# RajaeeKh/TriNerfLet

Measured on AMD Instinct MI355X. Metric: train rays/sec (whole node), higher is better.
Workload: dtype f16; 1 GPU; base: 3x32ch x 2048^2 planes, bior6.8 scale 32, hidden 64, 60000 rays/step/GPU, solid-sphere occupancy r=0.8 (re-imposed after each refresh), fp16 planes + fp16 MFMA MLP, fp32 masters, Adam+L1; GT colours = an analytic function of the ray direction (synthetic.target_colors), not a second seeded field's render; sample_budget_M=4769546, parallelism=ray-dp1

## Files before the change

include/trinerflet_hip.h:

```cpp
#ifndef TRINERFLET_HIP_H
#define TRINERFLET_HIP_H

#include <stdint.h>

#ifdef __cplusplus
extern "C" {
#endif

#define TNL_API __attribute__((visibility("default")))

TNL_API int tnl_abi_version(void);


TNL_API int tnl_near_far_from_aabb(const float *rays_o, const float *rays_d, const float *aabb,
                                   uint32_t N, float min_near, float *nears, float *fars,
                                   void *stream);

TNL_API int tnl_sph_from_ray(const float *rays_o, const float *rays_d, float radius, uint32_t N,
                             float *coords, void *stream);

TNL_API int tnl_morton3D(const int32_t *coords, uint32_t N, int32_t *indices, void *stream);

TNL_API int tnl_morton3D_invert(const int32_t *indices, uint32_t N, int32_t *coords, void *stream);

TNL_API int tnl_packbits(const float *grid, uint32_t N, float density_thresh, uint8_t *bitfield,
                         void *stream);
TNL_API int tnl_packbits_dev(const float *grid, uint32_t N, float density_thresh, const float *mean_density_dev,
                             uint8_t *bitfield, void *stream);

TNL_API int tnl_occupancy_bounds(const uint8_t *bitfield, uint32_t bytes_per_cascade, uint32_t cascades,
                                 int32_t *bounds, void *stream);
TNL_API int tnl_occupancy_row_extents(const uint8_t *bitfield, uint32_t bytes_per_cascade, uint32_t cascades, uint32_t H,
                                      float bound, uint32_t R, int32_t *ext, void *stream);

TNL_API int tnl_occupied_box(const uint8_t *bitfield, uint32_t bytes_per_cascade, uint32_t cascades, uint32_t H,
                             float bound, int32_t *bounds_scratch, float *box, void *stream);
TNL_API int tnl_clip_fars(const float *rays_o, const float *rays_d, const float *fars, const float *box, uint32_t N,
                          float *fars_out, void *stream);

TNL_API uint32_t tnl_march_rays_train_workspace(uint32_t N);
TNL_API uint32_t tnl_march_rays_train_workspace_rec(uint32_t N, uint32_t max_steps);

TNL_API int tnl_march_rays_train(const float *rays_o, const float *rays_d, const uint8_t *grid,
                                 float bound, float dt_gamma, uint32_t max_steps, uint32_t N,
                                 uint32_t C, uint32_t H, uint32_t M, const float *nears,
                                 const float *fars, float *xyzs, float *dirs, float *deltas,
                                 int32_t *rays, int32_t *counter, const float *noises,
                                 int32_t *workspace, uint32_t workspace_words, void *stream);
TNL_API int tnl_march_rays_train_binned(const float *rays_o, const float *rays_d, const uint8_t *grid,
                                 float bound, float dt_gamma, uint32_t max_steps, uint32_t N,
                                 uint32_t C, uint32_t H, uint32_t M, const float *nears,
                                 const float *fars, float *xyzs, float *dirs, float *deltas,
                                 int32_t *rays, int32_t *counter, const float *noises,
                                 int32_t *workspace, uint32_t workspace_words, uint32_t R, void *sort_workspace, void *stream);

TNL_API int tnl_march_count_form(int form);

TNL_API int tnl_march_emit_cap(int blocks);
TNL_API int tnl_plane_grad_fill_cap(int blocks);

TNL_API int tnl_composite_rays_train_forward(const float *sigmas, const float *rgbs,
                                             const float *deltas, const int32_t *rays, uint32_t M,
                                             uint32_t N, float T_thresh, float *weights_sum,
                                             float *depth, float *image, void *stream);

TNL_API int tnl_composite_rays_train_backward(const float *grad_weights_sum, const float *grad_image,
                                              const float *sigmas, const float *rgbs,
                                              const float *deltas, const int32_t *rays,
                                              const float *weights_sum, const float *image,
                                              uint32_t M, uint32_t N, float T_thresh,
                                              float *grad_sigmas, float *grad_rgbs, void *stream);

TNL_API int tnl_march_rays(uint32_t n_alive, uint32_t n_step, const int32_t *rays_alive,
                           const float *rays_t, const float *rays_o, const float *rays_d,
                           float bound, float dt_gamma, uint32_t max_steps, uint32_t C, uint32_t H,
                           const uint8_t *grid, const float *nears, const float *fars, float *xyzs,
                           float *dirs, float *deltas, const float *noises, void *stream);

TNL_API int tnl_composite_rays(uint32_t n_alive, uint32_t n_step, float T_thresh,
                               int32_t *rays_alive, float *rays_t, const float *sigmas,
                               const float *rgbs, const float *deltas, float *weights_sum,
                               float *depth, float *image, void *stream);

TNL_API int tnl_compact_rays(const int32_t *rays_alive, uint32_t n_alive, int32_t *rays_alive_out,
                             int32_t *n_out, int32_t *workspace, void *stream);

TNL_API int tnl_sh_encode_forward(const float *inputs, float *outputs, uint32_t B, uint32_t D,
                                  uint32_t C, float *dy_dx, void *stream);
TNL_API int tnl_sh_encode_backward(const float *grad, const float *inputs, uint32_t B, uint32_t D,
                                   uint32_t C, const float *dy_dx, float *grad_inputs, void *stream);


TNL_API int tnl_idwt_level_forward(const float *x, const float *yh, uint32_t S, uint32_t n,
                                   int wave, float *out, void *stream);

TNL_API int tnl_idwt_level_forward_half(const float *x, const float *yh, uint32_t S, uint32_t n,
                                        int wave, void *out_half, void *stream);

TNL_API int tnl_idwt_level_backward(const float *dout, uint32_t S, uint32_t n, int wave, float *dx,
                                    float *dyh, void *stream);

TNL_API int tnl_idwt_level_backward_adam(const float *dout, uint32_t S, uint32_t n, int wave, float *dx,
                                         float *p, float *m, float *v, float *ll_p, float *ll_m,
                                         float *ll_v, float step_size, float bias2_sqrt, float beta1,
                                         float beta2, float eps, float inv_scale,
                                         const float *inv_scale_dev, float l1_coef,
                                         const float *found_inf, float *abs_sum, void *stream);

TNL_API int tnl_planes_to_texel_major(const float *planes_cm, uint32_t C, uint32_t R, int half_out,
                                      void *planes_tm, void *stream);
TNL_API int tnl_planes_to_texel_major_win(const float *planes_cm, uint32_t C, uint32_t R, int half_out,
                                          void *planes_tm, const int32_t *roi, void *stream);
TNL_API int tnl_planes_half_to_texel_major(const void *planes_cm_half, uint32_t C, uint32_t R,
                                           void *planes_tm_half, void *stream);
TNL_API int tnl_planes_to_channel_major(const float *grad_tm, uint32_t C, uint32_t R, float *grad_cm,
                                        void *stream);

TNL_API int tnl_triplane_sample_forward(const void *planes_tm, int half_in, const float *xyz,
                                        float bound, uint32_t N, uint32_t C, uint32_t R, float *feats,
                                        void *stream);
TNL_API int tnl_triplane_sample_backward(const float *grad_feats, const float *xyz, float bound,
                                         uint32_t N, uint32_t C, uint32_t R, float *grad_tm,
                                         void *stream);

TNL_API int tnl_grid_sample_tm_forward(const void *planes_tm, int half_in, const float *grid, uint32_t N, uint32_t C,
                                       uint32_t CG, uint32_t R, float *feats, void *stream);
TNL_API int tnl_grid_sample_tm_backward(const void *planes_tm, int half_in, const float *grid,
                                        const float *grad_feats, uint32_t N, uint32_t C, uint32_t CG, uint32_t R,
                                        float *grad_tm, float *grad_grid, void *stream);

TNL_API uint32_t tnl_field_packed_bytes(uint32_t C, uint32_t Hd, uint32_t Hc);
TNL_API int tnl_field_pack(const float *W0, const float *W1, const float *W2, const float *W3,
                           const float *W4, uint32_t C, uint32_t Hd, uint32_t Hc, void *packed,
                           void *stream);
TNL_API uint64_t tnl_field_feats_save_bytes(uint32_t M, uint32_t C, uint32_t Hd);
TNL_API int tnl_field_forward(const void *planes_tm, int half_in, const float *xyz, const float *dirs,
                              float bound, uint32_t M, uint32_t C, uint32_t R, uint32_t Hd,
                              uint32_t Hc, const void *packed, float *sigma, float *rgb,
                              void *feats_save, const int32_t *m_actual, void *stream);
TNL_API uint64_t tnl_field_backward_workspace(uint32_t M, uint32_t C, uint32_t Hd, uint32_t Hc);
TNL_API int tnl_field_backward(const float *grad_sigma, const float *grad_rgb, const float *sigma,
                               const float *rgb, const void *feats_save, const float *xyz,
                               const float *dirs, float bound, uint32_t M, uint32_t C, uint32_t R,
                               uint32_t Hd, uint32_t Hc, const void *packed, float *grad_tm,
                               float *gradW, void *workspace, const int32_t *m_actual, void *dfeat_half,
                               void *stream);

TNL_API uint64_t tnl_plane_grad_binned_workspace(uint32_t M, uint32_t R);
TNL_API int tnl_plane_grad_binned(const void *dfeat_half, const float *xyz, float bound, uint32_t M,
                                  const int32_t *m_actual, uint32_t C, uint32_t R, float grad_scale,
                                  float *grad_out, int channel_major, int32_t *nonfinite_flag,
                                  void *workspace, void *stream);

TNL_API int tnl_plane_grad_sort_layout(uint32_t M, uint32_t R, int64_t *out);
TNL_API int tnl_plane_grad_sort(const float *xyz, float bound, uint32_t M, const int32_t *m_actual, uint32_t R,
                                void *workspace, void *stream);
TNL_API int tnl_plane_grad_sort_counted(const float *xyz, float bound, uint32_t M, const int32_t *m_actual,
                                        uint32_t R, void *workspace, void *stream);
TNL_API int tnl_plane_grad_reduce(const void *dfeat_half, const float *xyz, float bound, uint32_t M, uint32_t C,
                                  uint32_t R,
                                  float grad_scale, float *grad_out, int channel_major, int32_t *nonfinite_flag,
                                  const int32_t *roi, const void *workspace, void *stream);

TNL_API int tnl_idwt_level_forward_half_roi(const float *x, const float *yh, uint32_t S, uint32_t n, int wave,
                                            void *out_half, const int32_t *roi, void *stream);
TNL_API int tnl_planes_half_to_texel_major_roi(const void *planes_roi_half, uint32_t C, uint32_t R,
                                               void *planes_tm_half, const int32_t *roi, void *stream);
TNL_API int tnl_plane_grad_binned_roi(const void *dfeat_half, const float *xyz, float bound, uint32_t M,
                                      const int32_t *m_actual, uint32_t C, uint32_t R, float grad_scale,
                                      float *grad_out, int channel_major, int32_t *nonfinite_flag,
                                      const int32_t *roi, void *workspace, void *stream);
TNL_API int tnl_idwt_level_backward_roi(const float *dout_roi, uint32_t S, uint32_t n, int wave, float *dx,
                                        float *dyh, const int32_t *roi, void *stream);

TNL_API int tnl_adam_l1_step(float *p, float *grad, float *m, float *v, uint64_t n, float step_size,
                             float bias2_sqrt, float beta1, float beta2, float eps, float inv_scale,
                             const float *inv_scale_dev, float l1_coef, const float *found_inf,
                             float *abs_sum, int zero_grad, void *stream);
TNL_API int tnl_adam_l1_step_dev(float *p, float *grad, float *m, float *v, uint64_t n, float lr,
                                 const float *opt_step_dev, float beta1, float beta2, float eps, float inv_scale,
                                 const float *inv_scale_dev, float l1_coef, const float *found_inf,
// ... 122 lines not shown
```

trinerflet_amd/build.py:

```python
import glob
import os
import subprocess
import sys
from concurrent.futures import ThreadPoolExecutor

HERE = os.path.dirname(os.path.abspath(__file__))
CSRC = os.path.join(HERE, "csrc")
OBJ = os.path.join(HERE, "csrc", "_obj")
LIB = os.path.join(HERE, "libtrinerflet_hip.so")
HIPCC = os.environ.get("HIPCC", "/opt/rocm/bin/hipcc")
ARCH = "gfx950"
COMMON = ["--offload-arch=" + ARCH, "-O3", "-fPIC", "-std=c++17", "-fvisibility=hidden",
          "-Wall", "-Wno-unused-function", "-I", os.path.join(HERE, "..", "include")]
COMMON += os.environ.get("TNL_HIPCC_FLAGS", "").split()
MFMA_VGPR = ["-mllvm", "-amdgpu-mfma-vgpr-form=1"]
NO_SLP = ["-fno-slp-vectorize"]
PER_FILE = {"raymarch.hip": ["-ffp-contract=off"], "rays.hip": ["-ffp-contract=off"],
            "field_bwd.hip": MFMA_VGPR,
            "field_bwd_rows.hip": MFMA_VGPR + ["-mllvm", "-amdgpu-sched-strategy=max-ilp"], "field.hip": MFMA_VGPR, "scatter.hip": MFMA_VGPR,
            "render.hip": MFMA_VGPR + NO_SLP, "field_h128.hip": MFMA_VGPR + NO_SLP + ["-mllvm", "-amdgpu-sched-strategy=max-ilp"]}
for _spec in filter(None, os.environ.get("TNL_HIPCC_FILE_FLAGS", "").split(";")):
    _name, _flags = _spec.split(":", 1)
    PER_FILE[_name.strip()] = PER_FILE.get(_name.strip(), []) + _flags.split()
INCLUDES = {"field_h128.hip": ["field.hip"]}


def _newer(src, dst, extra=()):
    if not os.path.exists(dst):
        return True
    t = os.path.getmtime(dst)
    return any(os.path.getmtime(p) > t for p in (src, *extra))


def build(verbose=False, force=False):
    os.makedirs(OBJ, exist_ok=True)
    headers = glob.glob(os.path.join(CSRC, "*.h")) + glob.glob(os.path.join(HERE, "..", "include", "*.h"))
    srcs = sorted(glob.glob(os.path.join(CSRC, "*.hip")))
    jobs = []
    objs = []
    for s in srcs:
        o = os.path.join(OBJ, os.path.basename(s)[:-4] + ".o")
        objs.append(o)
        if force or _newer(s, o, headers + [os.path.join(CSRC, d) for d in INCLUDES.get(os.path.basename(s), [])]):
            jobs.append([HIPCC, *COMMON, *PER_FILE.get(os.path.basename(s), []), "-c", s, "-o", o])

    def run(cmd):
        if verbose:
            print(" ".join(cmd), flush=True)
        r = subprocess.run(cmd, capture_output=True, text=True)
        if r.returncode != 0:
            raise RuntimeError("hipcc failed:\n" + " ".join(cmd) + "\n" + r.stdout + r.stderr)
        if verbose and r.stderr.strip():
            print(r.stderr)

    with ThreadPoolExecutor(max_workers=4) as ex:
        list(ex.map(run, jobs))
    if jobs or not os.path.exists(LIB):
        run([HIPCC, "--offload-arch=" + ARCH, "-shared", "-fPIC", "-o", LIB, *objs])
    return LIB


if __name__ == "__main__":
    print(build(verbose=True, force="--force" in sys.argv))
```

trinerflet_amd/nerf/renderer.py:

```python
import math

import numpy as np
import torch
import torch.nn as nn

from .. import _lib as L
from .. import raymarching


def sample_pdf(bins, weights, n_samples, det=False):
    pdf = weights + 1e-5
    pdf = pdf / pdf.sum(-1, keepdim=True)
    cdf = torch.cat([torch.zeros_like(pdf[..., :1]), torch.cumsum(pdf, -1)], -1)
    if det:
        u = torch.linspace(0.5 / n_samples, 1.0 - 0.5 / n_samples, steps=n_samples, device=weights.device)
        u = u.expand(*cdf.shape[:-1], n_samples)
    else:
        u = torch.rand(*cdf.shape[:-1], n_samples, device=weights.device)
    u = u.contiguous()
    hi = torch.searchsorted(cdf, u, right=True)
    lo = (hi - 1).clamp(min=0)
    hi = hi.clamp(max=cdf.shape[-1] - 1)
    c_lo, c_hi = torch.gather(cdf, -1, lo), torch.gather(cdf, -1, hi)
    b_lo, b_hi = torch.gather(bins, -1, lo), torch.gather(bins, -1, hi)
    span = c_hi - c_lo
    span = torch.where(span < 1e-5, torch.ones_like(span), span)
    return b_lo + (u - c_lo) / span * (b_hi - b_lo)


class NeRFRenderer(nn.Module):
    def __init__(self, bound=1, cuda_ray=False, density_scale=1, min_near=0.2, density_thresh=0.01, bg_radius=-1,
                 **kwargs):
        super().__init__()
        self.bound = bound
        self.cascade = 1 + math.ceil(math.log2(bound))
        self.grid_size = 128
        self.density_scale = density_scale
        self.min_near = min_near
        self.density_thresh = density_thresh
        self.bg_radius = bg_radius
        self._march_count = None
        self._march_window = None
        self.use_occupancy_window = True
        self._occ_window_key = None
        self._occ_window = None
        aabb_train = torch.FloatTensor([-bound, -bound, -bound, bound, bound, bound])
        self.register_buffer('aabb_train', aabb_train)
        self.register_buffer('aabb_infer', aabb_train.clone())
        self.cuda_ray = cuda_ray
        if cuda_ray:
            self.register_buffer('density_grid', torch.zeros([self.cascade, self.grid_size ** 3]))
            self.register_buffer('density_bitfield',
                                 torch.zeros(self.cascade * self.grid_size ** 3 // 8, dtype=torch.uint8))
            self.mean_density = 0
            self.iter_density = 0
            self.register_buffer('step_counter', torch.zeros(16, 2, dtype=torch.int32))
            self.mean_count = 0
            self.local_step = 0
        self._morton_xyz = None

    def forward(self, x, d):
        raise NotImplementedError()

    def density(self, x):
        raise NotImplementedError()

    def color(self, x, d, mask=None, **kwargs):
        raise NotImplementedError()

    def reset_extra_state(self):
        if not self.cuda_ray:
            return
        self.density_grid.zero_()
        self.mean_density = 0
        self.iter_density = 0
        self.step_counter.zero_()
        self.mean_count = 0
        self.local_step = 0

    def run(self, rays_o, rays_d, num_steps=128, upsample_steps=128, bg_color=None, perturb=False, **kwargs):
        prefix = rays_o.shape[:-1]
        rays_o = rays_o.contiguous().view(-1, 3)
        rays_d = rays_d.contiguous().view(-1, 3)
        N, device = rays_o.shape[0], rays_o.device
        aabb = self.aabb_train if self.training else self.aabb_infer
        nears, fars = raymarching.near_far_from_aabb(rays_o, rays_d, aabb, self.min_near)
        nears, fars = nears.unsqueeze(-1), fars.unsqueeze(-1)
        z_vals = torch.linspace(0.0, 1.0, num_steps, device=device).unsqueeze(0).expand(N, num_steps)
        z_vals = nears + (fars - nears) * z_vals
        sample_dist = (fars - nears) / num_steps
        if perturb:
            z_vals = z_vals + (torch.rand(z_vals.shape, device=device) - 0.5) * sample_dist
        xyzs = rays_o.unsqueeze(-2) + rays_d.unsqueeze(-2) * z_vals.unsqueeze(-1)
        xyzs = torch.min(torch.max(xyzs, aabb[:3]), aabb[3:])
        dens = self.density(xyzs.reshape(-1, 3))
        sigma = dens['sigma'].view(N, num_steps)
        geo = dens['geo_feat'].view(N, num_steps, -1)
        if upsample_steps > 0:
            with torch.no_grad():
                d0 = z_vals[..., 1:] - z_vals[..., :-1]
                d0 = torch.cat([d0, sample_dist * torch.ones_like(d0[..., :1])], dim=-1)
                a0 = 1 - torch.exp(-d0 * self.density_scale * sigma)
                w0 = a0 * torch.cumprod(torch.cat([torch.ones_like(a0[..., :1]), 1 - a0 + 1e-15], dim=-1), dim=-1)[..., :-1]
                z_mid = z_vals[..., :-1] + 0.5 * d0[..., :-1]
                new_z = sample_pdf(z_mid, w0[:, 1:-1], upsample_steps, det=not self.training).detach()
                new_xyzs = rays_o.unsqueeze(-2) + rays_d.unsqueeze(-2) * new_z.unsqueeze(-1)
                new_xyzs = torch.min(torch.max(new_xyzs, aabb[:3]), aabb[3:])
            new_dens = self.density(new_xyzs.reshape(-1, 3))
            z_vals, order = torch.sort(torch.cat([z_vals, new_z], dim=1), dim=1)
            xyzs = torch.gather(torch.cat([xyzs, new_xyzs], dim=1), 1, order.unsqueeze(-1).expand(-1, -1, 3))
            sigma = torch.gather(torch.cat([sigma, new_dens['sigma'].view(N, upsample_steps)], dim=1), 1, order)
            geo = torch.cat([geo, new_dens['geo_feat'].view(N, upsample_steps, -1)], dim=1)
            geo = torch.gather(geo, 1, order.unsqueeze(-1).expand(-1, -1, geo.shape[-1]))
        deltas = z_vals[..., 1:] - z_vals[..., :-1]
        deltas = torch.cat([deltas, sample_dist * torch.ones_like(deltas[..., :1])], dim=-1)
        alphas = 1 - torch.exp(-deltas * self.density_scale * sigma)
        alphas_shifted = torch.cat([torch.ones_like(alphas[..., :1]), 1 - alphas + 1e-15], dim=-1)
        weights = alphas * torch.cumprod(alphas_shifted, dim=-1)[..., :-1]
        dirs = rays_d.view(-1, 1, 3).expand_as(xyzs)
        mask = weights > 1e-4
        rgbs = self.color(xyzs.reshape(-1, 3), dirs.reshape(-1, 3), mask=mask.reshape(-1),
                          geo_feat=geo.reshape(-1, geo.shape[-1]))
        rgbs = rgbs.view(N, -1, 3)
        weights_sum = weights.sum(dim=-1)
        ori_z_vals = ((z_vals - nears) / (fars - nears)).clamp(0, 1)
        depth = torch.sum(weights * ori_z_vals, dim=-1)
        image = torch.sum(weights.unsqueeze(-1) * rgbs, dim=-2)
        if bg_color is None:
            bg_color = 1
        image = image + (1 - weights_sum).unsqueeze(-1) * bg_color
        return {'depth': depth.view(*prefix), 'image': image.view(*prefix, 3), 'weights_sum': weights_sum}

    def run_cuda(self, rays_o, rays_d, dt_gamma=0, bg_color=None, perturb=False, force_all_rays=False,
                 max_steps=1024, T_thresh=1e-4, noises=None, **kwargs):
        prefix = rays_o.shape[:-1]
        rays_o = rays_o.contiguous().view(-1, 3)
        rays_d = rays_d.contiguous().view(-1, 3)
        N, device = rays_o.shape[0], rays_o.device
        nears, fars = raymarching.near_far_from_aabb(rays_o, rays_d,
                                                     self.aabb_train if self.training else self.aabb_infer,
                                                     self.min_near)
        fars_aabb = fars
        if getattr(self, "clip_far_to_occupancy", True):
            bf = self.density_bitfield
            key = (bf.data_ptr(), bf._version)
            if getattr(self, "_occ_box_key", None) != key:
                self._occ_box_cached = raymarching.occupied_box(bf, self.cascade, self.grid_size, self.bound)
                self._occ_box_key = key
            fars = raymarching.clip_fars(rays_o, rays_d, fars, self._occ_box_cached)
        if bg_color is None:
            bg_color = 1
        results = {}
        if self.training:
            counter = self.step_counter[self.local_step % 16]
            counter.zero_()
            self.local_step += 1
            xyzs, dirs, deltas, rays = raymarching.march_rays_train(
                rays_o, rays_d, self.bound, self.density_bitfield, self.cascade, self.grid_size, nears, fars, counter,
                self.mean_count, perturb, 128, force_all_rays, dt_gamma, max_steps, noises)
            self._march_count = counter
            self._march_window = self._occupancy_window() if hasattr(self, "_occupancy_window") else None
            try:
                sigmas, rgbs = self(xyzs, dirs)
            finally:
                self._march_count = self._march_window = None
            sigmas = self.density_scale * sigmas
            weights_sum, depth, image = raymarching.composite_rays_train(sigmas, rgbs, deltas, rays, T_thresh)
            image = image + (1 - weights_sum).unsqueeze(-1) * bg_color
            depth = torch.clamp(depth - nears, min=0) / (fars_aabb - nears)
            image = image.view(*prefix, 3)
            depth = depth.view(*prefix)
            results['weights_sum'] = weights_sum
        elif self._eval_render_mode(kwargs) == "kernel":
            weights_sum, depth, image = self._infer_render_kernel(rays_o, rays_d, nears, fars, dt_gamma, perturb,
                                                                  max_steps, T_thresh)
            image = image + (1 - weights_sum).unsqueeze(-1) * bg_color
            depth = torch.clamp(depth - nears, min=0) / (fars_aabb - nears)
            image = image.view(*prefix, 3)
            depth = depth.view(*prefix)
            weights_sum = weights_sum.view(*prefix)
# ... 33 lines not shown
            depth = torch.clamp(depth - nears, min=0) / (fars_aabb - nears)
            image = image.view(*prefix, 3)
            depth = depth.view(*prefix)
            weights_sum = weights_sum.view(*prefix)
        results['depth'] = depth
        results['image'] = image
        results['weights_sum'] = weights_sum
        return results

    RENDER_MODES = ("kernel", "device_loop", "host_loop")

    def _eval_render_mode(self, kwargs):
        mode = kwargs.get("render_mode")
        if mode is None:
            if "fused_render" in kwargs:
                mode = "kernel" if kwargs["fused_render"] else \
                    ("device_loop" if kwargs.get("device_loop", True) else "host_loop")
            elif "device_loop" in kwargs:
                mode = "device_loop" if kwargs["device_loop"] else "host_loop"
            elif "infer_min_step" in kwargs:
                mode = "device_loop"
            else:
                mode = "kernel"
        elif mode not in self.RENDER_MODES:
            raise ValueError(f"render_mode must be one of {self.RENDER_MODES}, got {mode!r}")
        elif mode != "device_loop" and kwargs.get("infer_min_step", 1) != 1:
            raise ValueError("infer_min_step is a knob of render_mode='device_loop'")
        if mode != "host_loop" and (not getattr(self, "_fused_ok", lambda: False)() or torch.is_grad_enabled()):
            mode = "host_loop"
        return mode

    def _infer_render_kernel(self, rays_o, rays_d, nears, fars, dt_gamma, perturb, max_steps, T_thresh):
        lib = L.lib()
        N, dev = rays_o.shape[0], rays_o.device
        weights_sum = torch.empty(N, dtype=torch.float32, device=dev)
        depth = torch.empty(N, dtype=torch.float32, device=dev)
        image = torch.empty(N, 3, dtype=torch.float32, device=dev)
        if N == 0:
            return weights_sum, depth, image
        enc = self.encoder
        tm = enc.get_planes_texel_major()
        packed = self.packed_weights()
        noises = torch.rand(N, dtype=torch.float32, device=dev) if perturb else None
        queue = torch.empty(1, dtype=torch.int32, device=dev)
        L.check(lib.tnl_render_rays(
            L.ptr(tm), L.i32(int(tm.dtype == torch.float16)), L.u32(enc.number_of_features), L.u32(enc.plane_resolution),
            L.u32(self.hidden_dim), L.u32(self.hidden_dim), L.ptr(packed), L.ptr(rays_o), L.ptr(rays_d), L.ptr(nears),
            L.ptr(fars), L.u32(N), L.ptr(self.density_bitfield), L.f32(self.bound), L.f32(dt_gamma), L.u32(max_steps),
            L.u32(self.cascade), L.u32(self.grid_size), L.f32(T_thresh), L.f32(float(self.density_scale)), L.ptr(noises),
            L.ptr(queue), L.ptr(weights_sum), L.ptr(depth), L.ptr(image), L.stream()), "render_rays")
        return weights_sum, depth, image

    def _infer_device_loop(self, rays_o, rays_d, nears, fars, dt_gamma, perturb, max_steps, T_thresh, poll=4,
                           min_step=1):
        lib = L.lib()
        N, dev = rays_o.shape[0], rays_o.device
        weights_sum = torch.zeros(N, dtype=torch.float32, device=dev)
        depth = torch.zeros(N, dtype=torch.float32, device=dev)
        image = torch.zeros(N, 3, dtype=torch.float32, device=dev)
        if N == 0:
            return weights_sum, depth, image
        state = torch.tensor([N, 0, 0, 0], dtype=torch.int32, device=dev)
        alive = [torch.arange(N, dtype=torch.int32, device=dev), torch.empty(N, dtype=torch.int32, device=dev)]
        rays_t = nears.clone()
        min_step = max(1, min(int(min_step), 8))
        cap = min_step * N + 128
        xyzs = torch.empty(cap, 3, dtype=torch.float32, device=dev)
        dirs = torch.empty(cap, 3, dtype=torch.float32, device=dev)
        deltas = torch.empty(cap, 2, dtype=torch.float32, device=dev)
        t_scratch = torch.empty(cap, dtype=torch.float32, device=dev)
        cws = torch.empty((N + 255) // 256 + 2, dtype=torch.int32, device=dev)
        noises = torch.rand(N, dtype=torch.float32, device=dev) if perturb else None
        rows = state[3:4]
        packed = self.packed_weights()

        def iteration(nz):
            L.check(lib.tnl_infer_plan(L.ptr(state), L.u32(N), L.u32(max_steps), L.u32(min_step), L.stream()),
                    "infer_plan")
            L.check(lib.tnl_march_rays_dev(
                L.ptr(state), L.u32(N), L.ptr(alive[0]), L.ptr(rays_t), L.ptr(rays_o), L.ptr(rays_d),
                L.f32(self.bound), L.f32(dt_gamma), L.u32(max_steps), L.u32(self.cascade), L.u32(self.grid_size),
                L.ptr(self.density_bitfield), L.ptr(fars), L.ptr(xyzs), L.ptr(dirs), L.ptr(deltas),
                L.ptr(nz), L.ptr(t_scratch), L.u32(cap), L.stream()), "march_rays_dev")
            sigmas, rgbs = self.field_rows(xyzs, dirs, rows, packed)
            if self.density_scale != 1:
                sigmas = self.density_scale * sigmas
            L.check(lib.tnl_composite_rays_dev(
                L.ptr(state), L.u32(N), L.f32(T_thresh), L.ptr(alive[0]), L.ptr(rays_t), L.ptr(sigmas),
                L.ptr(rgbs), L.ptr(deltas), L.ptr(weights_sum), L.ptr(depth), L.ptr(image), L.stream()),
                "composite_rays_dev")
            L.check(lib.tnl_compact_rays_dev(L.ptr(state), L.u32(N), L.ptr(alive[0]), L.ptr(alive[1]),
                                             L.ptr(cws), L.stream()), "compact_rays_dev")
            alive.reverse()

        def finished():
            n_alive, _, step, _ = state.tolist()
            return n_alive <= 0 or step >= max_steps

        it = 0
        while it < max_steps:
            for _ in range(poll):
                iteration(noises if it == 0 else None)
                it += 1
            if finished():
                break
        return weights_sum, depth, image

    def _cells(self):
        if self._morton_xyz is None or self._morton_xyz.device != self.density_bitfield.device:
            H = self.grid_size
            idx = torch.arange(H ** 3, dtype=torch.int32, device=self.density_bitfield.device)
            coords = raymarching.morton3D_invert(idx)
            self._morton_xyz = self._cell_centres(coords)
        return self._morton_xyz

    def _cell_centres(self, coords):
        den = torch.full((1,), float(self.grid_size - 1), dtype=torch.float32, device=coords.device)
        return 2 * coords.float() / den - 1

    @torch.no_grad()
    def mark_untrained_grid(self, poses, intrinsic, S=64):
        if not self.cuda_ray:
            return
        if isinstance(poses, np.ndarray):
            poses = torch.from_numpy(poses)
        fx, fy, cx, cy = intrinsic
        dev = self.density_grid.device
        poses = poses.to(dev).float()
        cells = self._cells()
        count = torch.zeros_like(self.density_grid)
        chunk = 64 ** 3
        for cas in range(self.cascade):
            bound = min(2 ** cas, self.bound)
            half_grid_size = bound / self.grid_size
            for c0 in range(0, cells.shape[0], chunk):
                world = (cells[c0:c0 + chunk] * (bound - half_grid_size)).unsqueeze(0)
                for head in range(0, poses.shape[0], S):
                    P = poses[head:head + S]
                    cam = (world - P[:, :3, 3].unsqueeze(1)) @ P[:, :3, :3]
                    mask = (cam[:, :, 2] > 0) \
                        & (torch.abs(cam[:, :, 0]) < cx / fx * cam[:, :, 2] + half_grid_size * 2) \
                        & (torch.abs(cam[:, :, 1]) < cy / fy * cam[:, :, 2] + half_grid_size * 2)
                    count[cas, c0:c0 + chunk] += mask.sum(0)
        self.density_grid[count == 0] = -1

    def _sigma_for_grid(self):
        stock = getattr(type(self), "_stock_density", None)
        fast = getattr(self, "density_sigma", None)
        if fast is not None and stock is not None and "density" not in self.__dict__ \
                and getattr(type(self).density, "__func__", type(self).density) is stock:
            return fast
        return lambda p_: self.density(p_)['sigma']

    @torch.no_grad()
    def update_extra_state(self, decay=0.95, S=128, shard=None, draws=None):
        if not self.cuda_ray:
            return
        dev = self.density_bitfield.device
        H = self.grid_size
        rank, world, gather = shard if shard is not None else (0, 1, None)
        tmp_grid = -torch.ones_like(self.density_grid)
        sigma_of = self._sigma_for_grid()

        def jitter(cas, xyzs):
            if draws is not None and draws.get("noise") is not None:
                return draws["noise"][cas].to(dev, torch.float32)
            return torch.rand_like(xyzs)
        if self.iter_density < 16:
            cells = self._cells()
            c0, c1 = cells.shape[0] * rank // world, cells.shape[0] * (rank + 1) // world
            for cas in range(self.cascade):
                bound = min(2 ** cas, self.bound)
                half_grid_size = bound / H
                xyzs = cells[c0:c1] * (bound - half_grid_size)
                xyzs = xyzs + (jitter(cas, xyzs) * 2 - 1) * half_grid_size
                dens = sigma_of(xyzs).reshape(-1).detach().float() * self.density_scale
                tmp_grid[cas] = dens if world == 1 else gather(dens)
        else:
            N = H ** 3 // 4 // world
            for cas in range(self.cascade):
                if draws is not None and draws.get("coords") is not None:
                    coords = draws["coords"][cas].to(dev)
                else:
                    coords = torch.randint(0, H, (N, 3), device=dev)
                indices = raymarching.morton3D(coords).long()
                running = torch.cumsum(self.density_grid[cas] > 0, 0)
                n_occ = running[-1]
                if draws is not None and draws.get("occ_k") is not None:
                    k = draws["occ_k"][cas].to(dev).long()
                else:
                    k = (torch.rand(N, device=dev, dtype=torch.float64) * n_occ).long().clamp_(max=(n_occ - 1).clamp(min=0))
                occ_indices = torch.searchsorted(running, k + 1)
                occ_indices = torch.where(n_occ > 0, occ_indices, torch.full_like(occ_indices, H ** 3))
                occ_coords = raymarching.morton3D_invert(occ_indices.clamp(max=H ** 3 - 1))
                indices = torch.cat([indices, occ_indices], dim=0)
                coords = torch.cat([coords, occ_coords], dim=0)
                xyzs = self._cell_centres(coords)
                bound = min(2 ** cas, self.bound)
                half_grid_size = bound / H
                xyzs = xyzs * (bound - half_grid_size)
                xyzs = xyzs + (jitter(cas, xyzs) * 2 - 1) * half_grid_size
                dens = sigma_of(xyzs).reshape(-1).detach().float() * self.density_scale
                tmp_c = -torch.ones(H ** 3 + 1, dtype=tmp_grid.dtype, device=dev)
                if world == 1:
                    tmp_c.scatter_reduce_(0, indices, dens, reduce="amax", include_self=True)
                else:
                    tmp_c.scatter_reduce_(0, gather(indices), gather(dens), reduce="amax", include_self=True)
                tmp_grid[cas] = tmp_c[:H ** 3]
        valid_mask = (self.density_grid >= 0) & (tmp_grid >= 0)
        self.density_grid.copy_(torch.where(valid_mask, torch.maximum(self.density_grid * decay, tmp_grid),
                                            self.density_grid))
        mean_dev = torch.mean(self.density_grid.clamp(min=0)).reshape(1).float()
        self.iter_density += 1
        L.check(L.lib().tnl_packbits_dev(L.ptr(self.density_grid), L.u32(self.density_bitfield.numel()),
                                         L.f32(self.density_thresh), L.ptr(mean_dev), L.ptr(self.density_bitfield),
                                         L.stream()), "packbits_dev")
        self.density_bitfield[:0].zero_()
        self._occ_box_key = None
        total_step = min(16, self.local_step)
        csum = self.step_counter[:total_step, 0].sum().reshape(1).double() if total_step > 0 else mean_dev.double() * 0
        mean_h, csum_h = torch.cat([mean_dev.double(), csum]).tolist()
        self.mean_density = mean_h
        if total_step > 0:
            self.mean_count = int(csum_h / total_step)
        self.local_step = 0

    def render(self, rays_o, rays_d, staged=False, max_ray_batch=4096, **kwargs):
        _run = self.run_cuda if self.cuda_ray else self.run
        B, N = rays_o.shape[:2]
        device = rays_o.device
        if staged and not self.cuda_ray:
            depth = torch.empty((B, N), device=device)
            image = torch.empty((B, N, 3), device=device)
            for b in range(B):
                for head in range(0, N, max_ray_batch):
                    tail = min(head + max_ray_batch, N)
                    res = _run(rays_o[b:b + 1, head:tail], rays_d[b:b + 1, head:tail], **kwargs)
                    depth[b:b + 1, head:tail] = res['depth']
                    image[b:b + 1, head:tail] = res['image']
            return {'depth': depth, 'image': image}
        return _run(rays_o, rays_d, **kwargs)
```

trinerflet_amd/train.py:

```python
from ._step.common import (C_, D, F_, L, _Flat, _IDWTLevel, _StepState, _ToTexelMajor, dist, half_roi_into_texel_major,
                           half_to_texel_major, idwt_level_half, idwt_level_half_roi, lr_factor, math, np, occupancy, raymarching,
                           torch, types)
from ._step.graph import GraphMixin
from ._step.optimiser import OptimiserMixin
from ._step.planes import PlanesMixin
from ._step.prefetch import PrefetchMixin
from ._step.window import WindowMixin


class TrainStep(WindowMixin, PlanesMixin, OptimiserMixin, PrefetchMixin, GraphMixin):
    def __init__(self, model, lr=1e-2, wavelet_regularization=0.4, iters=30000, warmup_steps=0,
                 betas=(0.9, 0.99), eps=1e-15, fp16=True, update_extra_interval=16, background_color=0.0,
                 max_steps=1024, dt_gamma=0.0, T_thresh=1e-4, init_scale=65536.0, growth_interval=2000,
                 dist_mode=None, process_group=None, single_rank_collectives=False, binned=True, fuse_adam=False, use_roi=True, tune_placement=None,
                 defer_adam=None, deterministic=False, live_bands=True, overlap_exchange=0, graph=False,
                 min_wavelet_resolution_to_learn=-1, grad_transport="fp32"):
        enc = model.encoder
        assert model.cuda_ray, "TrainStep drives the cuda_ray renderer (every README configuration)"
        if not model._fused_ok():
            raise NotImplementedError("TrainStep needs a configuration the fused field kernel is built for")
        self.base_res = int(getattr(enc, "wavelet_base_resolution", 0) or 0)
        self.crop_k = 2 * int(getattr(enc, "planes_features_wavelet_pad", 0) or 0)
        self.model, self.enc = model, enc
        self.C, self.R, self.H = enc.number_of_features, enc.plane_resolution, model.hidden_dim
# ... 46 lines not shown
            def _reloaded(module, incompatible):
                ts_ = me_()
                if ts_ is not None:
                    ts_._frozen_abs = None
            self._ld_hook = model.register_load_state_dict_post_hook(_reloaded)
        self.placement = None
        if (tune_placement if tune_placement is not None else self.coef.total >= 64_000_000) and self.coef.total > 0:
            self.placement = self.coef.tune_placement(self._time_adam_pass)
        self.defer_adam = (defer_adam if defer_adam is not None else self.coef.total >= 32_000_000) and self._rect_ok
        self._ring = torch.zeros(16 * 4, dtype=torch.float32, device=dev)
        self._ring_sums = torch.zeros(16, dtype=torch.float32, device=dev)
        self._pending = 0
        self._live = None
        self._live_bands = None
        self.last_live_bands = None
        self._band_cache = {}
        self._row_ext = None
        self._rects_roi = None
        self.last_live = None
        self._defer_ctx = None
        self.deferred_reg = torch.zeros((), dtype=torch.float32, device=dev)
        self.deferred_steps = 0
        import weakref
        me = weakref.ref(self)

        def _flush_before_state_dict(module, prefix, keep_vars):
            ts = me()
            if ts is not None and ts.model is module:
                ts.flush_deferred()
        self._sd_hook = model.register_state_dict_pre_hook(_flush_before_state_dict)
        self.deferred_flushes = 0
        self.last_flush_records = 0
        self.clip_far_in_order = False
        self._occ_box = None
        self.scale = torch.full((1,), init_scale if fp16 else 1.0, dtype=torch.float32, device=dev)
        self.growth_tracker = torch.zeros(1, dtype=torch.int32, device=dev)
        self.growth_interval = growth_interval
        self.opt_steps = torch.zeros(1, dtype=torch.float32, device=dev)
        self.abs_sum = torch.zeros(1, dtype=torch.float32, device=dev)
        self.nonfinite = torch.zeros(1, dtype=torch.int32, device=dev)
        self.inv_scale = torch.ones(1, dtype=torch.float32, device=dev)
        self.last = {}
        self.section_names = None
        self._mark_seq = 0
        self.overlap_march = True
        self.overlap_exchange = overlap_exchange if overlap_exchange == "auto" else int(overlap_exchange)
        self._auto_plan = None
        assert grad_transport in ("fp32", "bf16")
        self.grad_transport = grad_transport
        self._comm = None
        self.live_col_align = 32
        self.live_bands = live_bands
        self._side = None
        self._prefetched = None
        self.graph = bool(graph)
        self._graphs = {}
        self._graph_key = None
        self._graph_pool = None
        self._graph_in = None
        self._cap_stream = None
        self._graph_done = None
        self._capturing = False
        self._lr_dev = None
        self.graph_replays = 0
        self.graph_captures = 0
        self._key_captures = self._key_replays = self._wasted_keys = 0
        self.graph_auto_disabled = False
        self._stale_params = self._stale_moments = False
        self.prefetch_at = "bwd"
        self.side_count_form = 1
        if __import__("os").environ.get("TNL_SIDE_COUNT_FORM") is not None:
            self.side_count_form = int(__import__("os").environ["TNL_SIDE_COUNT_FORM"])
        if __import__("os").environ.get("TNL_PREFETCH_AT") is not None:
            self.prefetch_at = __import__("os").environ["TNL_PREFETCH_AT"]
        n_cu = torch.cuda.get_device_properties(self.dev).multi_processor_count if torch.cuda.is_available() else 256
        self.side_caps = (2 * n_cu, n_cu) if 3 * self.C * self.R * self.R >= (1 << 27) else (0, 0)
        if __import__("os").environ.get("TNL_SIDE_CAPS"):
            self.side_caps = tuple(int(v) for v in __import__("os").environ["TNL_SIDE_CAPS"].split(","))
        self.post_refresh = None
        self.section_events = None
        self.pg = process_group
        self.world = dist.get_world_size(process_group) if (dist_mode and dist.is_initialized()) else 1
        if dist_mode == "auto":
            dist_mode = "sharded" if (3 * self.C) % max(self.world, 1) == 0 else "allreduce"
            if overlap_exchange == 0:
                self.overlap_exchange = "auto"
        self.rank = dist.get_rank(process_group) if self.world > 1 else 0
        self.multi = self.world > 1 or bool(single_rank_collectives and dist_mode and dist.is_initialized())
        if self.multi and self.world == 1:
            D.force_collectives(process_group)
            import weakref
            weakref.finalize(self, D.force_collectives, process_group, False)
        self.dist_mode = dist_mode if self.multi else None
        if self.dist_mode == "sharded":
            assert (3 * self.C) % self.world == 0, "3*channels must be divisible by the world size"
        if self.multi:
            g3 = model.grid_size ** 3
            assert g3 % self.world == 0 and (g3 // 4) % self.world == 0, \
                f"grid_size^3 / 4 = {g3 // 4} candidate cells cannot be split evenly over {self.world} ranks"

    def _mark(self, name):
        self._mark_seq += 1
        if self.section_events is not None and (self.section_names is None or name in self.section_names):
            ev = torch.cuda.Event(enable_timing=True)
            ev.record()
            self.section_events.append((name, ev, self._mark_seq))

    def section_times(self, stat="mean"):
        if not self.section_events:
            return {}
        vals = {}
        prev = None
        for name, ev, seq in self.section_events:
            if name != "begin" and prev is not None and prev[1] == seq - 1:
                vals.setdefault(name, []).append(prev[0].elapsed_time(ev))
            prev = (ev, seq)
        if stat == "median":
            return {k: float(np.median(v)) for k, v in vals.items()}
        return {k: sum(v) / len(v) for k, v in vals.items()}

    def step(self, rays_o, rays_d, gt_rgb, noises=None, n_global_rays=None, bg_color=None, next_rays=None):
        self.model.train()
        N = rays_o.shape[0]
        st = _StepState(rays_o=rays_o, rays_d=rays_d, gt_rgb=gt_rgb, noises=noises, bg_color=bg_color, next_rays=next_rays,
                        N=N, n_glob=n_global_rays if n_global_rays is not None else N * self.world,
                        refresh=self.update_extra_interval > 0 and self.global_step % self.update_extra_interval == 0)
        if self.graph and self._graph_eligible(st):
            return self._graph_step(st)
        self._mark("begin")
        self._stage_pickup(st)
        self._stage_planes(st)
        self._stage_march(st)
        self._stage_render(st)
        self._stage_backward(st)
        self._stage_optimise(st)
        return st.loss

    def _stage_pickup(self, st):
        model = self.model
        st.side, st.marched = None, None
        pre = self._prefetched
        if pre is not None and not st.refresh and self._prefetch_matches(pre[0], st.rays_o, st.rays_d, st.noises):
            self._prefetched = None
            st.marched, st.side = pre[1], self._side
        else:
            self._drop_prefetch()
            if self.overlap_march and not st.refresh and model.mean_count > 0:
                st.marched, st.side = self._march_on_side(st.rays_o, st.rays_d, st.noises), self._side

    def _stage_planes(self, st):
        model = self.model
        if self._roi_request is not None:
            self._roi = self._finish_roi()
        if self._pending and (st.refresh or not self._roi_valid):
            self.flush_deferred()
            self._mark("adam_catchup")
        if self.use_roi and not st.refresh and not self._roi_valid:
            self._roi, self._roi_valid = self._compute_roi(), True
        st.tm = self.rebuild_planes(roi=self.use_roi and not st.refresh)
        self._mark("idwt_fwd")
        if st.refresh:
            if self.multi:
                model.update_extra_state(shard=(self.rank, self.world, lambda t: D.all_gather_slices(t, self.pg)))
                mc = torch.tensor([float(model.mean_count)], dtype=torch.float64, device=self.dev)
                dist.all_reduce(mc, group=self.pg)
                model.mean_count = int(mc.item() / self.world)
            else:
                model.update_extra_state()
            if self.post_refresh is not None:
                self.post_refresh()
            self._occ_box = None
            if self.use_roi:
                self._request_roi()
                self._roi_valid = True
            self._mark("grid_refresh")

    def _stage_march(self, st):
        model, R = self.model, self.R
        st.packed = F_.pack_weights(*self.Ws, self.C, self.H)
        st.sort_beside = False
        if st.side is None:
            if self.overlap_march and self.binned and R % 32 == 0 and model.mean_count > 0:
                if self._side is None:
                    self._side = torch.cuda.Stream()
                st.marched = self._march(st.rays_o, st.rays_d, st.noises, sort_stream=self._side, clip=self.clip_far_in_order)
                st.sort_beside = True
            else:
                st.marched = self._march(st.rays_o, st.rays_d, st.noises, clip=self.clip_far_in_order)
        marched, (ev_march, st.ev_sort) = st.marched
        if st.side is not None:
            torch.cuda.current_stream().wait_event(ev_march)
        st.counter, st.xyzs, st.dirs, st.deltas, st.rays, st.sort_ws = marched
        st.M = st.xyzs.shape[0]
        self._mark("march")

    def _stage_render(self, st):
        model, lib = self.model, L.lib()
        C, R, H, N, M = self.C, self.R, self.H, st.N, st.M
        sigma, st.rgb, st.feats = F_.field_forward(st.tm, st.xyzs, st.dirs, st.packed, float(model.bound), C, R, H,
                                                   save_feats=True, m_actual=st.counter)
        st.sigma_field = sigma
        if model.density_scale != 1:
            sigma = sigma * model.density_scale
        st.sigma = sigma
        self._mark("field_fwd")
        st.ws = torch.empty(N, dtype=torch.float32, device=self.dev)
        st.depth = torch.empty(N, dtype=torch.float32, device=self.dev)
        st.image = torch.empty(N, 3, dtype=torch.float32, device=self.dev)
        L.check(lib.tnl_composite_rays_train_forward(L.ptr(sigma), L.ptr(st.rgb), L.ptr(st.deltas), L.ptr(st.rays), L.u32(M),
                                                     L.u32(N), L.f32(self.T_thresh), L.ptr(st.ws), L.ptr(st.depth),
                                                     L.ptr(st.image), L.stream()), "composite_rays_train_forward")
        bg = self.bg if st.bg_color is None else st.bg_color
        st.pred = torch.empty(N, 3, dtype=torch.float32, device=self.dev)
        st.g_pred = torch.empty(N, 3, dtype=torch.float32, device=self.dev)
        st.g_ws = torch.empty(N, dtype=torch.float32, device=self.dev)
        st.mse_local = torch.empty((), dtype=torch.float32, device=self.dev)
        L.check(lib.tnl_step_prologue(L.ptr(self.scale), L.ptr(self.inv_scale), L.ptr(self.abs_sum),
                                      L.ptr(self.nonfinite), L.ptr(st.mse_local), L.ptr(self.mlp.grad),
                                      L.u32(self.mlp.grad.numel()), L.stream()), "step_prologue")
        bg_rays = bg.to(torch.float32).contiguous() if torch.is_tensor(bg) else None
        L.check(lib.tnl_mse_loss(L.ptr(st.image), L.ptr(st.ws), L.ptr(st.gt_rgb.contiguous()),
                                 L.f32(0.0 if bg_rays is not None else bg), L.ptr(bg_rays), L.u32(N),
                                 L.f32(1.0 / (3.0 * st.n_glob)), L.ptr(self.scale), L.ptr(st.pred), L.ptr(st.g_pred),
                                 L.ptr(st.g_ws), L.ptr(st.mse_local), L.stream()), "mse_loss")
        self._mark("composite_fwd_loss")

    def _stage_backward(self, st):
        model, lib = self.model, L.lib()
        C, R, H, N, M = self.C, self.R, self.H, st.N, st.M
        g_sigma = torch.empty(M, dtype=torch.float32, device=self.dev)
        g_rgb = torch.empty(M, 3, dtype=torch.float32, device=self.dev)
        L.check(lib.tnl_composite_rays_train_backward(L.ptr(st.g_ws), L.ptr(st.g_pred), L.ptr(st.sigma), L.ptr(st.rgb),
                                                      L.ptr(st.deltas), L.ptr(st.rays), L.ptr(st.ws), L.ptr(st.image), L.u32(M),
                                                      L.u32(N), L.f32(self.T_thresh), L.ptr(g_sigma), L.ptr(g_rgb),
                                                      L.stream()), "composite_rays_train_backward")
        if model.density_scale != 1:
            g_sigma = g_sigma * model.density_scale
        self._mark("composite_bwd")
        if self._roi_request is not None:
            self._roi = self._finish_roi()
        st.roi = self._roi if (self.use_roi and self.binned and R % 32 == 0) else None
        if self.binned and R % 32 == 0:
            if st.roi is None:
                st.g_cm = torch.empty(3, C, R, R, dtype=torch.float32, device=self.dev)
            else:
                st.g_cm = torch.empty(3 * C, st.roi[7], st.roi[6], dtype=torch.float32, device=self.dev)
            dfeat = torch.empty(3, M, C, dtype=torch.float16, device=self.dev)
            F_.field_backward(g_sigma, g_rgb, st.sigma_field, None, st.feats, st.xyzs, st.dirs, st.packed, float(model.bound),
                              C, R, H, st.g_cm, self.mlp.grad, m_actual=st.counter, dfeat=dfeat)
            self._mark("field_bwd")
            if self.prefetch_at == "bwd":
                self._prefetch_next(st.next_rays)
            if st.side is not None or st.sort_beside:
                torch.cuda.current_stream().wait_event(st.ev_sort)
            if self.deterministic:
                F_.order_tile_lists(st.sort_ws, R, st.xyzs.shape[0])
            st.scattered = False
            bands = self._exchange_bands(st.roi)
            if bands is None:
                F_.plane_grad_reduce(st.sort_ws, dfeat, st.xyzs, float(model.bound), C, R, st.g_cm, channel_major=True,
                                     nonfinite_flag=self.nonfinite, roi=self._roi10() if st.roi is not None else None)
            else:
                if self._comm is None:
                    self._comm = torch.cuda.Stream()
                main = torch.cuda.current_stream()
                parts, waits = [], []
                for y0, hb in bands:
                    buf = torch.empty(3 * C, hb, st.roi[6], dtype=torch.float32, device=self.dev)
                    sub = list(st.roi)
                    sub[3:6] = [oy + y0 for oy in st.roi[3:6]]
                    sub[7] = hb
                    F_.plane_grad_reduce(st.sort_ws, dfeat, st.xyzs, float(model.bound), C, R, buf, channel_major=True,
                                         nonfinite_flag=self.nonfinite, roi=sub + [C, 0])
                    self._comm.wait_stream(main)
                    with torch.cuda.stream(self._comm):
                        part, wait = D.reduce_scatter_slices_async(buf, self.pg if self.multi else None, self.grad_transport)
                    buf.record_stream(self._comm)
                    parts.append(part)
                    waits.append(wait)
                for w in waits:
                    w()
                main.wait_stream(self._comm)
                s0, s1 = self._slice_range() if self.multi else (0, 3 * C)
                st.g_cm = torch.cat([p_[: s1 - s0] if not self.multi else p_ for p_ in parts], dim=1)
                st.scattered = self.multi
            if self.prefetch_at == "reduce":
                self._prefetch_next(st.next_rays)
            self._mark("plane_grad_binned")
            st.grad_tm = None
        else:
            st.g_cm = None
            st.grad_tm = torch.zeros(3, R, R, C, dtype=torch.float32, device=self.dev)
            F_.field_backward(g_sigma, g_rgb, st.sigma_field, None, st.feats, st.xyzs, st.dirs, st.packed, float(model.bound),
                              C, R, H, st.grad_tm, self.mlp.grad, m_actual=st.counter)
            self._mark("field_bwd")
            self._prefetch_next(st.next_rays)

    def _stage_optimise(self, st):
        lib = L.lib()
        lr_t = self.lr * lr_factor(self.global_step, self.iters, self.warmup)
        l1 = self.lam / (self.J * self.coef_numel) if (self.J > 0 and self.lam > 0) else 0.0
        inv_scale = self.inv_scale
        if self.multi:
            dist.all_reduce(self.mlp.grad, group=self.pg)
        if st.g_cm is not None:
            found_inf = self._scaler_probe(self.mlp.grad, None, self.nonfinite)
# ... 85 lines not shown
```

Baseline: 9.517 million rays/s.

## Move occupancy grid refresh into HIP kernels with deferred host readbacks

```diff
diff --git a/include/trinerflet_hip.h b/include/trinerflet_hip.h
--- a/include/trinerflet_hip.h
+++ b/include/trinerflet_hip.h
@@ -27,6 +27,14 @@
                          void *stream);
 TNL_API int tnl_packbits_dev(const float *grid, uint32_t N, float density_thresh, const float *mean_density_dev,
                              uint8_t *bitfield, void *stream);
+
+TNL_API int tnl_grid_candidates(const void *coords, int coords_i64, const int64_t *occ_k, const double *occ_u,
+                                const int64_t *running, const float *noise, uint32_t N, uint32_t n, uint32_t H,
+                                uint32_t first, float scale, float half, int32_t *indices, float *xyzs, void *stream);
+TNL_API int tnl_grid_scatter_max(const int32_t *indices, const float *dens, float density_scale, uint32_t n,
+                                 uint32_t H3, float *tmp, void *stream);
+TNL_API int tnl_grid_update(float *grid, const float *const *src, uint32_t cascades, uint32_t H3, float src_scale,
+                            float decay, void *stream);
 
 TNL_API int tnl_occupancy_bounds(const uint8_t *bitfield, uint32_t bytes_per_cascade, uint32_t cascades,
                                  int32_t *bounds, void *stream);
diff --git a/trinerflet_amd/build.py b/trinerflet_amd/build.py
--- a/trinerflet_amd/build.py
+++ b/trinerflet_amd/build.py
@@ -16,6 +16,8 @@
 MFMA_VGPR = ["-mllvm", "-amdgpu-mfma-vgpr-form=1"]
 NO_SLP = ["-fno-slp-vectorize"]
 PER_FILE = {"raymarch.hip": ["-ffp-contract=off"], "rays.hip": ["-ffp-contract=off"],
+            "grid_update.hip": ["-ffp-contract=off"],
+
             "field_bwd.hip": MFMA_VGPR,
             "field_bwd_rows.hip": MFMA_VGPR + ["-mllvm", "-amdgpu-sched-strategy=max-ilp"], "field.hip": MFMA_VGPR, "scatter.hip": MFMA_VGPR,
             "render.hip": MFMA_VGPR + NO_SLP, "field_h128.hip": MFMA_VGPR + NO_SLP + ["-mllvm", "-amdgpu-sched-strategy=max-ilp"]}
diff --git a/trinerflet_amd/csrc/grid_update.hip b/trinerflet_amd/csrc/grid_update.hip
--- /dev/null
+++ b/trinerflet_amd/csrc/grid_update.hip
@@ -0,0 +1,126 @@
+#include <hip/hip_runtime.h>
+#include <stdint.h>
+
+#include "../../include/trinerflet_hip.h"
+#include "march_device.h"
+
+#pragma clang fp contract(off)
+
+namespace {
+
+inline uint32_t cdiv_(uint32_t a, uint32_t b) { return (a + b - 1) / b; }
+
+__global__ void __launch_bounds__(256)
+k_grid_candidates(const void* __restrict__ coords, int coords_i64, const int64_t* __restrict__ occ_k,
+                  const double* __restrict__ occ_u, const int64_t* __restrict__ running, const float* __restrict__ noise,
+                  uint32_t N, uint32_t n, uint32_t H, uint32_t H3, uint32_t first, float scale, float half,
+                  int32_t* __restrict__ indices, float* __restrict__ xyzs) {
+  const uint32_t i = threadIdx.x + blockIdx.x * blockDim.x;
+  if (i >= n) return;
+  uint32_t c[3];
+  if (coords == nullptr) {
+    const uint32_t cell = first + i;
+    c[0] = morton3D_invert_(cell); c[1] = morton3D_invert_(cell >> 1); c[2] = morton3D_invert_(cell >> 2);
+  } else if (i < N) {
+#pragma unroll
+    for (int a = 0; a < 3; a++)
+      c[a] = coords_i64 ? (uint32_t)reinterpret_cast<const int64_t*>(coords)[(size_t)i * 3 + a]
+                        : (uint32_t)reinterpret_cast<const int32_t*>(coords)[(size_t)i * 3 + a];
+    indices[i] = (int32_t)morton3D_(c[0], c[1], c[2]);
+  } else {
+    const uint32_t j = i - N;
+    const int64_t n_occ = running[H3 - 1];
+    int64_t k;
+    if (occ_k != nullptr) {
+      k = occ_k[j];
+    } else {
+      k = (int64_t)(occ_u[j] * (double)n_occ);
+      const int64_t top = n_occ > 0 ? n_occ - 1 : 0;
+      if (k > top) k = top;
+    }
+    uint32_t lo = 0, hi = H3;
+    while (lo < hi) {
+      const uint32_t mid = lo + ((hi - lo) >> 1);
+      if (running[mid] < k + 1) lo = mid + 1; else hi = mid;
+    }
+    if (n_occ <= 0) lo = H3;
+    indices[i] = (int32_t)lo;
+    const uint32_t cell = lo < H3 ? lo : H3 - 1;
+    c[0] = morton3D_invert_(cell); c[1] = morton3D_invert_(cell >> 1); c[2] = morton3D_invert_(cell >> 2);
+  }
+  const float den = (float)(H - 1);
+#pragma unroll
+  for (int a = 0; a < 3; a++) {
+    const float centre = 2.f * (float)(int32_t)c[a] / den - 1.f;
+    const float jitter = (noise[(size_t)i * 3 + a] * 2.f - 1.f) * half;
+    xyzs[(size_t)i * 3 + a] = centre * scale + jitter;
+  }
+}
+
+__global__ void __launch_bounds__(256)
+k_grid_scatter_max(const int32_t* __restrict__ indices, const float* __restrict__ dens, float density_scale, uint32_t n,
+                   uint32_t H3, float* __restrict__ tmp) {
+  const uint32_t i = threadIdx.x + blockIdx.x * blockDim.x;
+  if (i >= n) return;
+  const uint32_t idx = (uint32_t)indices[i];
+  if (idx > H3) return;
+  const float v = dens[i] * density_scale;
+  uint32_t bits = __float_as_uint(v);
+  if (v != v) bits = 0x7fc00000u;
+  if ((bits >> 31) == 0) atomicMax(reinterpret_cast<int*>(tmp + idx), (int)bits);
+  else atomicMin(reinterpret_cast<unsigned int*>(tmp + idx), bits);
+}
+
+constexpr int GRID_UPDATE_MAX_CASCADES = 8;
+struct GridSrc { const float* p[GRID_UPDATE_MAX_CASCADES]; };
+
+__global__ void __launch_bounds__(256)
+k_grid_update(float* __restrict__ grid, GridSrc src, float src_scale, float decay, uint32_t H3) {
+  const float* __restrict__ s = src.p[blockIdx.y];
+  float* __restrict__ g = grid + (size_t)blockIdx.y * H3;
+  for (uint32_t i = threadIdx.x + blockIdx.x * blockDim.x; i < H3; i += gridDim.x * blockDim.x) {
+    const float old = g[i], t = s[i] * src_scale;
+    if (old >= 0.f && t >= 0.f) g[i] = fmaxf(old * decay, t);
+  }
+}
+
+}
+
+extern "C" {
+
+int tnl_grid_candidates(const void* coords, int coords_i64, const int64_t* occ_k, const double* occ_u,
+                        const int64_t* running, const float* noise, uint32_t N, uint32_t n, uint32_t H, uint32_t first,
+                        float scale, float half, int32_t* indices, float* xyzs, void* stream) {
+  if (n == 0) return 0;
+  const uint64_t H3 = (uint64_t)H * H * H;
+  if (H < 2 || H3 >= (1ull << 31) || noise == nullptr || xyzs == nullptr) return (int)hipErrorInvalidValue;
+  if (coords == nullptr) {
+    if ((uint64_t)first + n > H3) return (int)hipErrorInvalidValue;
+  } else if (n != 2 * (uint64_t)N || running == nullptr || indices == nullptr || (occ_k == nullptr) == (occ_u == nullptr)) {
+    return (int)hipErrorInvalidValue;
+  }
+  hipLaunchKernelGGL(k_grid_candidates, dim3(cdiv_(n, 256)), dim3(256), 0, (hipStream_t)stream, coords, coords_i64, occ_k,
+                     occ_u, running, noise, N, n, H, (uint32_t)H3, first, scale, half, indices, xyzs);
+  return (int)hipGetLastError();
+}
+
+int tnl_grid_scatter_max(const int32_t* indices, const float* dens, float density_scale, uint32_t n, uint32_t H3,
+                         float* tmp, void* stream) {
+  if (n == 0) return 0;
+  hipLaunchKernelGGL(k_grid_scatter_max, dim3(cdiv_(n, 256)), dim3(256), 0, (hipStream_t)stream, indices, dens,
+                     density_scale, n, H3, tmp);
+  return (int)hipGetLastError();
+}
+
+int tnl_grid_update(float* grid, const float* const* src, uint32_t cascades, uint32_t H3, float src_scale, float decay,
+                    void* stream) {
+  if (cascades == 0 || H3 == 0) return 0;
+  if (cascades > (uint32_t)GRID_UPDATE_MAX_CASCADES) return (int)hipErrorInvalidValue;
+  GridSrc s = {};
+  for (uint32_t c = 0; c < cascades; c++) s.p[c] = src[c];
+  const uint32_t blocks = cdiv_(H3, 256 * 4) < 2048u ? cdiv_(H3, 256 * 4) : 2048u;
+  hipLaunchKernelGGL(k_grid_update, dim3(blocks, cascades), dim3(256), 0, (hipStream_t)stream, grid, s, src_scale, decay, H3);
+  return (int)hipGetLastError();
+}
+
+}
diff --git a/trinerflet_amd/nerf/renderer.py b/trinerflet_amd/nerf/renderer.py
--- a/trinerflet_amd/nerf/renderer.py
+++ b/trinerflet_amd/nerf/renderer.py
@@ -1,3 +1,4 @@
+import ctypes
 import math
 
 import numpy as np
@@ -26,6 +27,34 @@
     span = c_hi - c_lo
     span = torch.where(span < 1e-5, torch.ones_like(span), span)
     return b_lo + (u - c_lo) / span * (b_hi - b_lo)
+
+
+class _HostScalar:
+
+    def __init__(self, dev_tensor, convert):
+        self._convert = convert
+        self._buf = torch.empty(1, dtype=dev_tensor.dtype, pin_memory=True)
+        self._buf.copy_(dev_tensor.reshape(1), non_blocking=True)
+        self._event = torch.cuda.Event()
+        self._event.record(torch.cuda.current_stream(dev_tensor.device))
+        self._value = None
+
+    def get(self):
+        if self._event is not None:
+            self._event.synchronize()
+            self._value = self._convert(self._buf[0].item())
+            self._buf = self._event = self._convert = None
+        return self._value
+
+    def __deepcopy__(self, memo):
+        return self.get()
+
+    def __reduce__(self):
+        return (_identity, (self.get(),))
+
+
+def _identity(v):
+    return v
 
 
 class NeRFRenderer(nn.Module):
@@ -365,8 +394,111 @@
             return fast
         return lambda p_: self.density(p_)['sigma']
 
+    def _host_attr(self, name, default=0):
+        v = self.__dict__.get(name, default)
+        if isinstance(v, _HostScalar):
+            v = self.__dict__[name] = v.get()
+        return v
+
+    mean_count = property(lambda self: self._host_attr("_mean_count"),
+                          lambda self, v: self.__dict__.__setitem__("_mean_count", v))
+    mean_density = property(lambda self: self._host_attr("_mean_density"),
+                            lambda self, v: self.__dict__.__setitem__("_mean_density", v))
+
     @torch.no_grad()
-    def update_extra_state(self, decay=0.95, S=128, shard=None, draws=None):
+    def begin_count_readback(self):
+        if not self.cuda_ray:
+            return
+        total_step = min(16, self.local_step)
+        self._count_readback = None
+        if total_step > 0:
+            csum = self.step_counter[:total_step, 0].sum().reshape(1)
+            self._count_readback = (self.local_step, _HostScalar(csum, lambda s, t=total_step: int(float(s) / t)))
+
+    @torch.no_grad()
+    def update_extra_state(self, decay=0.95, S=128, shard=None, draws=None, impl="hip"):
+        if impl not in ("hip", "torch"):
+            raise ValueError(f"update_extra_state: impl must be 'hip' or 'torch', not {impl!r}")
+        if not self.cuda_ray:
+            return
+        if shard is not None or impl == "torch":
+            self._count_readback = None
+            return self._update_extra_state_torch(decay, S, shard, draws)
+        dev = self.density_bitfield.device
+        H, lib = self.grid_size, L.lib()
+        H3 = H ** 3
+        rb = self.__dict__.get("_count_readback")
+        if rb is None or rb[0] != self.local_step:
+            self.begin_count_readback()
+            rb = self._count_readback
+        self._count_readback = None
+        self.mean_density
+        sigma_of = self._sigma_for_grid()
+
+        def candidates(cas, n, coords=None, occ_k=None, occ_u=None, running=None, indices=None, first=0):
+            xyzs = torch.empty(n, 3, dtype=torch.float32, device=dev)
+            if draws is not None and draws.get("noise") is not None:
+                noise = draws["noise"][cas].to(dev, torch.float32).contiguous()
+            else:
+                noise = torch.rand_like(xyzs)
+            assert noise.numel() == 3 * n
+            bound = min(2 ** cas, self.bound)
+            half = bound / H
+            L.check(lib.tnl_grid_candidates(L.ptr(coords), L.i32(coords is not None and coords.dtype == torch.int64),
+                                            L.ptr(occ_k), L.ptr(occ_u), L.ptr(running), L.ptr(noise), L.u32(n // 2), L.u32(n),
+                                            L.u32(H), L.u32(first), L.f32(bound - half), L.f32(half), L.ptr(indices),
+                                            L.ptr(xyzs), L.stream()), "grid_candidates")
+            return xyzs
+
+        def sigma(xyzs):
+            return sigma_of(xyzs).reshape(-1).detach().float().contiguous()
+        if self.iter_density < 16:
+            src = [sigma(candidates(cas, H3)) for cas in range(self.cascade)]
+            src_scale = self.density_scale
+        else:
+            N = H3 // 4
+            tmp = torch.full((self.cascade, H3 + 1), -1.0, dtype=torch.float32, device=dev)
+            for cas in range(self.cascade):
+                if draws is not None and draws.get("coords") is not None:
+                    coords = draws["coords"][cas].to(dev)
+                    if coords.dtype not in (torch.int32, torch.int64):
+                        coords = coords.int()
+                    coords = coords.contiguous()
+                else:
+                    coords = torch.randint(0, H, (N, 3), device=dev)
+                running = torch.cumsum(self.density_grid[cas] > 0, 0)
+                occ_k = occ_u = None
+                if draws is not None and draws.get("occ_k") is not None:
+                    occ_k = draws["occ_k"][cas].to(dev).long().contiguous()
+                else:
+                    occ_u = torch.rand(N, device=dev, dtype=torch.float64)
+                assert coords.shape == (N, 3) and (occ_k if occ_k is not None else occ_u).shape == (N,)
+                indices = torch.empty(2 * N, dtype=torch.int32, device=dev)
+                dens = sigma(candidates(cas, 2 * N, coords, occ_k, occ_u, running, indices))
+                assert dens.numel() == 2 * N
+                L.check(lib.tnl_grid_scatter_max(L.ptr(indices), L.ptr(dens), L.f32(self.density_scale), L.u32(2 * N),
+                                                 L.u32(H3), L.ptr(tmp[cas]), L.stream()), "grid_scatter_max")
+            src, src_scale = [tmp[cas] for cas in range(self.cascade)], 1.0
+        for s in src:
+            assert s.numel() >= H3 and s.dtype == torch.float32
+        for c0 in range(0, self.cascade, 8):
+            part = src[c0:c0 + 8]
+            ptrs = (ctypes.c_void_p * len(part))(*[s.data_ptr() for s in part])
+            L.check(lib.tnl_grid_update(L.ptr(self.density_grid[c0]), ptrs, L.u32(len(part)), L.u32(H3), L.f32(src_scale),
+                                        L.f32(decay), L.stream()), "grid_update")
+        mean_dev = torch.mean(self.density_grid.clamp(min=0)).reshape(1).float()
+        self.iter_density += 1
+        L.check(lib.tnl_packbits_dev(L.ptr(self.density_grid), L.u32(self.density_bitfield.numel()),
+                                     L.f32(self.density_thresh), L.ptr(mean_dev), L.ptr(self.density_bitfield),
+                                     L.stream()), "packbits_dev")
+        self.density_bitfield[:0].zero_()
+        self._occ_box_key = None
+        self.mean_density = _HostScalar(mean_dev, float)
+        if rb is not None:
+            self.mean_count = rb[1]
+        self.local_step = 0
+
+    def _update_extra_state_torch(self, decay, S, shard, draws):
         if not self.cuda_ray:
             return
         dev = self.density_bitfield.device
diff --git a/trinerflet_amd/train.py b/trinerflet_amd/train.py
--- a/trinerflet_amd/train.py
+++ b/trinerflet_amd/train.py
@@ -222,6 +222,8 @@
         model = self.model
         if self._roi_request is not None:
             self._roi = self._finish_roi()
+        if st.refresh and not self.multi:
+            model.begin_count_readback()
         if self._pending and (st.refresh or not self._roi_valid):
             self.flush_deferred()
             self._mark("adam_catchup")
```

After: 9.513 million rays/s. No clear change (-0.0%).
